# kehanxuuu/vspg-pbrt-v4

Measured on AMD Instinct MI355X. Metric: Mpaths/sec on 1920x1080 homogeneous fog; relMSE vs CPU ref at equal spp, higher is better.
Workload: dtype f32; 1 GPU; fog-box 1920x1080, guidedvolpathvspg vspguiding=true (primary-ray VSP; App. F options), 1 spp per step per GPU, independent sampler seed 0, maxdepth 5

## Files before the change

### vspg-pbrt-v4_amd/csrc/vspg_device.h

```cpp
#pragma once
#include <hip/hip_runtime.h>
#include <stdint.h>

#include "../../include/vspg.h"
#include "vspg_arith.h"
#include "vspg_libm.h"

#define VDEV __device__ __forceinline__
#ifdef VSPG_WF_DEBUG
__device__ unsigned int g_dbg_err[8];
#define VSPG_DBG_CHECK(cond, bit) do { if (!(cond)) atomicOr(&g_dbg_err[0], 1u << (bit)); } while (0)
#else
#define VSPG_DBG_CHECK(cond, bit)
#endif
#ifdef VSPG_NOINLINE_LEAVES
#define VLEAF __device__ __attribute__((noinline))
#else
#define VLEAF __device__ __forceinline__
#endif

VSPG_NS_BEGIN

#ifdef VSPG_PROFILE
enum { PS_INTERSECT = 0, PS_HASHRNG, PS_DIST_GUIDED, PS_DIST_PLAIN, PS_SURF_PRE, PS_NEE, PS_NEE_TR, PS_VOL_SAMPLE,
// ... 360 lines not shown
    V3 local = V3{clampf(sinTheta, -1, 1) * cosPhi, clampf(sinTheta, -1, 1) * sinPhi, clampf(cosTheta, -1, 1)};
    *pdf = henyey_greenstein(cosTheta, g);
    return f.from_local(local);
}
VDEV V3 sample_henyey_greenstein(V3 wo, float g, float u0, float u1, float *pdf) {
    float st, ct;
    float phi = hg_pre(g, u0, u1, &st, &ct);
    float sinPhi, cosPhi;
    sincosf_(phi, &sinPhi, &cosPhi);
    return hg_post(wo, g, st, ct, sinPhi, cosPhi, pdf);
}
VDEV float cos_hemi_pre(float u0, float u1, float *r, bool *degenerate) {
    float ox = 2 * u0 - 1, oy = 2 * u1 - 1;
    *degenerate = (ox == 0 && oy == 0);
    const bool xmajor = __builtin_fabsf(ox) > __builtin_fabsf(oy);
    const float q = (xmajor ? oy : ox) / (xmajor ? ox : oy);
    *r = xmajor ? ox : oy;
    const float t = kPiOver4 * q;
    return xmajor ? t : kPiOver2 - t;
}
VDEV V3 cos_hemi_post(float r, bool degenerate, float sinT, float cosT) {
    float dx = degenerate ? 0.f : r * cosT;
    float dy = degenerate ? 0.f : r * sinT;
    float z = safe_sqrt(1 - sqr(dx) - sqr(dy));
    return V3{dx, dy, z};
}
VDEV V3 sample_cosine_hemisphere(float u0, float u1) {
    float r;
    bool deg;
    float theta = cos_hemi_pre(u0, u1, &r, &deg);
    float sinTheta, cosTheta;
    sincosf_(theta, &sinTheta, &cosTheta);
    return cos_hemi_post(r, deg, sinTheta, cosTheta);
}

struct P3i {
    V3 lo, hi;
    VDEV V3 mid() const { return V3{(lo.x + hi.x) / 2, (lo.y + hi.y) / 2, (lo.z + hi.z) / 2}; }
    VDEV V3 err() const { return V3{(hi.x - lo.x) / 2, (hi.y - lo.y) / 2, (hi.z - lo.z) / 2}; }
};
VDEV P3i p3i_exact(V3 p) { return P3i{p, p}; }
VDEV void interval_ve(float v, float e, float *lo, float *hi) {
    float l = next_float_down(v - e), h = next_float_up(v + e);
    *lo = e == 0 ? v : l;
    *hi = e == 0 ? v : h;
}
VDEV P3i p3i_from_err(V3 p, V3 e) {
    P3i r;
    interval_ve(p.x, e.x, &r.lo.x, &r.hi.x);
    interval_ve(p.y, e.y, &r.lo.y, &r.hi.y);
    interval_ve(p.z, e.z, &r.lo.z, &r.hi.z);
    return r;
}
VDEV float offset_axis(float po, float off) {
    const uint32_t ui = f2b(po), os = f2b(off) & 0x80000000u;
    uint32_t r = ui + ((uint32_t)((int32_t)(ui ^ os) >> 31) | 1u);
    r = (ui << 1) == 0u ? (os | 1u) : r;
    const bool keep = !__builtin_islessgreater(off, 0.f) || (ui ^ os) == 0x7f800000u;
    return b2f(keep ? ui : r);
}
VDEV V3 offset_ray_origin(P3i pi, V3 n, V3 w) {
    float d = dot(vabs(n), pi.err());
    V3 offset = n * d;
    if (dot(w, n) < 0) offset = -offset;
    V3 po = pi.mid() + offset;
    return V3{offset_axis(po.x, offset.x), offset_axis(po.y, offset.y), offset_axis(po.z, offset.z)};
}
VDEV V3 medium_ray_origin(P3i pi) {
    const V3 n = V3{0.f, 0.f, 0.f};
    const float d = dot(n, pi.err());
    return pi.mid() + n * d;
}

#define VSPG_GLOBAL_AS __attribute__((address_space(1)))
struct DQuad {
    float p00[3], p10[3], p01[3], p11[3], e1[3], e2[3];
    float n[3], dpdu_n[3], perr[3];
    float inv_l1, inv_l2, area;
    float Kd[3], Le[3];
    int32_t two_sided, is_light, has_lobes;
    int32_t flags;
};
enum { SURF_INTERFACE = 1, SURF_IFACE_SHIFT = 1 };
enum { kIsectStepsMask = 3, kIsectUvSwapped = 4, kIsectAxisAligned = 8, kIsectAxisShift = 4 };
struct IsectRec {
    float f[14];
    int32_t kind;
    int32_t axes;
};
inline int isect_rec_build(IsectRec *rec, const float *n, const float *p00, const float *e1, const float *e2, float inv_l1, float inv_l2, int cur) {
    int ax[3];
    const float *vec[3] = {n, e1, e2};
    for (int j = 0; j < 3; ++j) {
        int nz = 0;
        ax[j] = -1;
        for (int k = 0; k < 3; ++k)
            if (vec[j][k] != 0) { nz++; ax[j] = k; }
        if (nz != 1) ax[j] = -1;
    }
    const int an = ax[0], a1 = ax[1], a2 = ax[2];
    for (int k = 0; k < 14; ++k) rec->f[k] = 0;
    int frame = 0;
    bool swapped = false;
    if (an >= 0 && an <= 2 && a1 >= 0 && a2 >= 0 && an != a1 && an != a2 && a1 != a2 && (n[an] == 1.0f || n[an] == -1.0f)) {
        swapped = a1 != (an + 1) % 3;
        const int au = swapped ? a2 : a1, av = swapped ? a1 : a2;
        frame = an;
        rec->kind = 1;
        rec->f[0] = n[an]; rec->f[1] = p00[an]; rec->f[2] = p00[au]; rec->f[3] = p00[av];
        rec->f[4] = swapped ? e2[a2] : e1[a1]; rec->f[5] = swapped ? e1[a1] : e2[a2];
        rec->f[6] = swapped ? inv_l2 : inv_l1; rec->f[7] = swapped ? inv_l1 : inv_l2;
    } else {
        rec->kind = 0;
        for (int k = 0; k < 3; ++k) { rec->f[k] = n[k]; rec->f[3 + k] = p00[k]; rec->f[6 + k] = e1[k]; rec->f[9 + k] = e2[k]; }
        rec->f[12] = inv_l1; rec->f[13] = inv_l2;
    }
    if (cur < 0 || cur > 2) cur = 0;
    rec->axes = ((frame - cur + 3) % 3) | (swapped ? kIsectUvSwapped : 0) | (rec->kind == 1 ? kIsectAxisAligned : 0) | (frame << kIsectAxisShift);
    return frame;
}
constexpr int kPlaneChunk = 4;
struct RectPlanes {
    float c[3][kPlaneChunk];
    uint32_t listed, always;
    uint32_t order[4];
};
static_assert(VSPG_MAX_QUADS <= 16 && 3 * kPlaneChunk + VSPG_MAX_QUADS < 32, "a record index is 4 bits of RectPlanes::order, a position one bit of 32");
inline void rect_planes_build(RectPlanes *T, const IsectRec *recs, int n) {
    *T = RectPlanes{};
    uint32_t done = 0;
    int count[3] = {0, 0, 0};
    auto place = [&](int pos, int i) { T->order[(pos - 1) >> 3] |= (uint32_t)i << (4 * ((pos - 1) & 7)); };
    for (int i = 0; i < n; ++i) {
        const int a = (recs[i].axes >> kIsectAxisShift) & 3;
        if (!(recs[i].axes & kIsectAxisAligned) || a > 2 || count[a] == kPlaneChunk) continue;
        const int pos = kPlaneChunk * a + count[a] + 1;
        T->c[a][count[a]++] = recs[i].f[1];
        T->listed |= 1u << pos;
        place(pos, i);
        done |= 1u << i;
    }
    int pos = 3 * kPlaneChunk + 1;
    for (int i = 0; i < n; ++i)
        if (!(done >> i & 1u)) {
            T->always |= 1u << pos;
            place(pos++, i);
        }
}
struct DField {
    int32_t n_nodes, n_regions;
    const VspgKdNode *nodes;
    const VspgFieldRegion *regions;
    const float *aux;
    const float4 *lobes;
};
constexpr int kMaxLights = VSPG_MAX_QUADS + VSPG_MAX_INFINITE_LIGHTS + VSPG_MAX_POINT_LIGHTS;
struct DLightNode {
    float bmin[3], bmax[3], w[3];
    float phi, cosTheta_o, cosTheta_e;
    int32_t twoSided;
    uint32_t child_or_light;
    int32_t is_leaf;
};
struct DLightSampler {
    int32_t mode;
    int32_t n_nodes, n_inf, n_alias;
    DLightNode nodes[2 * kMaxLights];
    int32_t inf_light[VSPG_MAX_INFINITE_LIGHTS];
    uint32_t bit_trail[kMaxLights];
    float alias_p[kMaxLights], alias_q[kMaxLights];
    int32_t alias_i[kMaxLights];
    int32_t light_of_quad[VSPG_MAX_QUADS];
};
struct DTri {
    float p0[3], nx;
    float p1[3], ny;
    float p2[3], nz;
    float dpdu_n[3];
    int32_t id;
    float Kd[3];
    int32_t flags;
};
struct DSphere {
    float m[12], mi[12];
    float radius, thetaZMin, thetaZMax, phiMax;
    float Kd[3];
    int32_t flip, has_lobes, flags;
};
struct DBvh4Node {
    float lox[4], loy[4], loz[4], hix[4], hiy[4], hiz[4];
    int32_t child[4];
    int32_t pad[4];
};
static_assert(sizeof(DBvh4Node) == 128, "one node = eight 16-byte loads");
constexpr int32_t kBvhAbsent = (int32_t)0x80000000;
constexpr int kBvhStack = 48;
struct PixelWindow {
    int32_t x0, y0, x1, y1;
};
__host__ __device__ __forceinline__ int win_tile_x0(const PixelWindow &w) { return w.x0 >> 3; }
__host__ __device__ __forceinline__ int win_tile_y0(const PixelWindow &w) { return w.y0 >> 3; }
__host__ __device__ __forceinline__ int win_tiles_x(const PixelWindow &w) { return ((w.x1 + 7) >> 3) - (w.x0 >> 3); }
__host__ __device__ __forceinline__ int win_tiles_y(const PixelWindow &w) { return ((w.y1 + 7) >> 3) - (w.y0 >> 3); }
__host__ __device__ __forceinline__ bool win_has(const PixelWindow &w, int px, int py) { return px >= w.x0 && px < w.x1 && py >= w.y0 && py < w.y1; }
struct DEnvLight {
    int32_t res;
    float integral;
    float m[9], mi[9];
    float sum_L[3];
    const float *texels;
    const float *func;
    const float *cdf;
    const float *mfunc;
    const float *mcdf;
};
struct DPointLight {
    int32_t type;
    float pos[3];
    float I[3];
    float mi[12];
    float cosFalloffEnd, cosFalloffStart;
    float axis[3];
};
struct DScene {
    int32_t n_quads, n_lights;
    int32_t n_tris, n_bvh_nodes;
    int32_t n_spheres, has_boundaries, camera_in_medium, pad_b;
    VspgCamera cam;
    int32_t medium_type;
    float sigma_a[3], sigma_s[3], Le[3], g;
// ... 84 lines not shown
static_assert(VSPG_MAX_QUADS <= kSpherePrim, "rectangle indices lie below the first sphere primitive");
VDEV bool is_sphere(int prim) { return prim >= kSpherePrim; }
VDEV int sphere_of(int prim) { return prim - kSpherePrim; }

VDEV bool beyond(float num, float denom, float tMax) {
    return __builtin_fabsf(num) > tMax * __builtin_fabsf(denom) * 1.000001f;
}
VDEV float comp(V3 v, int axis) { return axis == 0 ? v.x : (axis == 1 ? v.y : v.z); }
VDEV void swap_regs(float &a, float &b) { asm("v_swap_b32 %0, %1" : "+v"(a), "+v"(b)); }
VDEV void here(float a, float b, float c, float d) { asm volatile("" : : "s"(a), "s"(b), "s"(c), "s"(d)); }
VDEV void rect_frame(V3 &o, V3 &d, int steps) {
#pragma nounroll
    for (int k = steps & kIsectStepsMask; k > 0; --k) {
        swap_regs(o.x, o.y);
        swap_regs(o.y, o.z);
        swap_regs(d.x, d.y);
        swap_regs(d.y, d.z);
    }
}
VDEV bool rect_hit_uv(const IsectRec &r, V3 o, V3 d, float tMax, float *tHit, float *uHit, float *vHit) {
    float num, denom, u, v, t;
    bool cand;
    if (r.axes & kIsectAxisAligned) {
        denom = d.x;
        num = r.f[1] - o.x;
        cand = (int32_t)(__builtin_bit_cast(uint32_t, num) ^ __builtin_bit_cast(uint32_t, denom)) >= 0;
        cand = cand & !beyond(num, denom, tMax);
#if defined(__HIP_DEVICE_COMPILE__)
        const bool some = __ballot(cand) != 0ull;
#elif defined(VSPG_RECT_VOTE_TAKEN)
        const bool some = true;
#else
        const bool some = cand;
#endif
        if (!some) return false;
        t = num / denom;
        cand = cand & (t > 0) & (t < tMax);
        float pu = o.y + d.y * t, pv = o.z + d.z * t;
        u = ((pu - r.f[2]) * r.f[4]) * r.f[6];
        v = ((pv - r.f[3]) * r.f[5]) * r.f[7];
    } else {
        V3 n = V3{r.f[0], r.f[1], r.f[2]}, p00 = V3{r.f[3], r.f[4], r.f[5]};
        denom = dot(n, d);
        num = dot(n, p00 - o);
        cand = ((num > 0) & (denom > 0)) | ((num < 0) & (denom < 0));
        cand = cand & !beyond(num, denom, tMax);
#if defined(__HIP_DEVICE_COMPILE__)
        const bool some = __ballot(cand) != 0ull;
#elif defined(VSPG_RECT_VOTE_TAKEN)
        const bool some = true;
#else
        const bool some = cand;
#endif
        if (!some) return false;
        t = num / denom;
        cand = cand & (t > 0) & (t < tMax);
        V3 p = o + d * t;
        V3 rel = p - p00;
        u = dot(rel, V3{r.f[6], r.f[7], r.f[8]}) * r.f[12];
        v = dot(rel, V3{r.f[9], r.f[10], r.f[11]}) * r.f[13];
    }
    cand = cand & !((u < 0) | (u > 1) | (v < 0) | (v > 1));
    *tHit = t;
    *uHit = u;
    *vHit = v;
    return cand;
}
VDEV bool rects_closest(const IsectRec *recs, int n, V3 o, V3 d, float tMax, float *tBest, int *iBest, float *uBest, float *vBest) {
    bool hit = false;
    float bt = tMax, bu = 0, bv = 0;
    int bi = 0;
    V3 fo = o, fd = d;
    for (int i = 0; i < n; ++i) {
        const IsectRec &r = recs[i];
        float t, u, v;
        rect_frame(fo, fd, r.axes);
        const bool h = rect_hit_uv(r, fo, fd, bt, &t, &u, &v);
        const bool swapped = (r.axes & kIsectUvSwapped) != 0;
        hit = hit | h;
        bt = h ? t : bt;
        bi = h ? i : bi;
        bu = h ? (swapped ? v : u) : bu;
        bv = h ? (swapped ? u : v) : bv;
    }
    *tBest = bt;
    *iBest = bi;
    *uBest = bu;
    *vBest = bv;
    return hit;
}
VDEV bool rects_any(const IsectRec *recs, int n, V3 o, V3 d, float tMax) {
    bool any = false;
    V3 fo = o, fd = d;
    for (int i = 0; i < n; ++i) {
        const IsectRec &r = recs[i];
        float t, u, v;
        rect_frame(fo, fd, r.axes);
        any = any | rect_hit_uv(r, fo, fd, tMax, &t, &u, &v);
    }
    return any;
}
VDEV uint32_t plane_vote(float c, float oa, float da, float thr, uint32_t bit) {
    const float num = c - oa;
    const bool same = (int32_t)(__builtin_bit_cast(uint32_t, num) ^ __builtin_bit_cast(uint32_t, da)) >= 0, within = !(__builtin_fabsf(num) > thr);
#if defined(__HIP_DEVICE_COMPILE__)
    const bool some = (__builtin_amdgcn_ballot_w64(same) & __builtin_amdgcn_ballot_w64(within)) != 0ull;
#elif defined(VSPG_RECT_VOTE_TAKEN)
    const bool some = true;
#else
    const bool some = same & within;
#endif
    return some ? bit : 0u;
}
VDEV uint32_t axis_votes(const float *c, uint32_t listed, int a, float oa, float da, float tMax) {
    const float thr = tMax * __builtin_fabsf(da) * 1.000001f;
    static_assert(kPlaneChunk == 4, "one four-word load");
    const float p[kPlaneChunk] = {c[0], c[1], c[2], c[3]};
    here(p[0], p[1], p[2], p[3]);
    uint32_t m = 0;
#pragma unroll
    for (int k = 0; k < kPlaneChunk; ++k) {
        const uint32_t bit = 2u << (kPlaneChunk * a + k);
        if (!(listed & bit)) return m;
        m |= plane_vote(p[k], oa, da, thr, bit);
    }
    return m;
}
VDEV bool rects_any_planes(const RectPlanes &T, const IsectRec *recs, V3 o, V3 d, float tMax) {
    const uint32_t listed = T.listed;
    uint32_t mask = T.always;
    mask |= axis_votes(T.c[0], listed, 0, o.x, d.x, tMax);
    mask |= axis_votes(T.c[1], listed, 1, o.y, d.y, tMax);
    mask |= axis_votes(T.c[2], listed, 2, o.z, d.z, tMax);
    if (mask == 0) return false;
    bool any = false;
    V3 fo = o, fd = d;
    int cur = 0;
#pragma nounroll
    while (mask != 0) {
        const int pos = __builtin_ctz(mask) - 1;
        mask &= mask - 1;
        const IsectRec &r = recs[(T.order[pos >> 3] >> (4 * (pos & 7))) & 15u];
        const int frame = (r.axes >> kIsectAxisShift) & 3;
        float t, u, v;
        rect_frame(fo, fd, frame - cur + (frame < cur ? 3 : 0));
        cur = frame;
        any = any | rect_hit_uv(r, fo, fd, tMax, &t, &u, &v);
    }
    return any;
}
VDEV bool quad_hit_uv(const DQuad &q, V3 o, V3 d, float tMax, float *tHit, float *uHit, float *vHit) {
    V3 n = ld3(q.n), p00 = ld3(q.p00);
    float denom = dot(n, d);
    float num = dot(n, p00 - o);
    bool cand = (num > 0 && denom > 0) || (num < 0 && denom < 0);
    if (!cand) return false;
    float t = num / denom;
    if (!(t > 0) || !(t < tMax)) return false;
    V3 p = o + d * t;
    V3 rel = p - p00;
    float u = dot(rel, ld3(q.e1)) * q.inv_l1;
    float v = dot(rel, ld3(q.e2)) * q.inv_l2;
    if (u < 0 || u > 1 || v < 0 || v > 1) return false;
    *tHit = t;
    *uHit = u;
    *vHit = v;
// ... 196 lines not shown
        const float *row = S.mi + 4 * k;
        const float v = (row[0] * ro.x + row[1] * ro.y) + (row[2] * ro.z + row[3]);
        const float e = g3 * (__builtin_fabsf(row[0] * ro.x) + __builtin_fabsf(row[1] * ro.y) + __builtin_fabsf(row[2] * ro.z) + __builtin_fabsf(row[3]));
        oi[k] = ivl_from_err(v, e);
        const float ev = g3 * (__builtin_fabsf(row[0] * rd.x) + __builtin_fabsf(row[1] * rd.y) + __builtin_fabsf(row[2] * rd.z));
        const float vv = row[0] * rd.x + row[1] * rd.y + row[2] * rd.z;
        di[k] = ivl_from_err(vv, ev);
    }
    const Ivl a = ivl_add(ivl_add(ivl_sqr(di[0]), ivl_sqr(di[1])), ivl_sqr(di[2]));
    const Ivl b = ivl_fmul(2.f, ivl_add(ivl_add(ivl_mul(di[0], oi[0]), ivl_mul(di[1], oi[1])), ivl_mul(di[2], oi[2])));
    const Ivl c = ivl_sub(ivl_add(ivl_add(ivl_sqr(oi[0]), ivl_sqr(oi[1])), ivl_sqr(oi[2])), ivl_sqr(ivl_x(S.radius)));
    const Ivl f = ivl_div(b, ivl_fmul(2.f, a));
    const Ivl v0 = ivl_sub(oi[0], ivl_mul(f, di[0])), v1 = ivl_sub(oi[1], ivl_mul(f, di[1])), v2 = ivl_sub(oi[2], ivl_mul(f, di[2]));
    const Ivl length = ivl_sqrt(ivl_add(ivl_add(ivl_sqr(v0), ivl_sqr(v1)), ivl_sqr(v2)));
    const Ivl discrim = ivl_mul(ivl_mul(ivl_fmul(4.f, a), ivl_add(ivl_x(S.radius), length)), ivl_sub(ivl_x(S.radius), length));
    if (discrim.lo < 0) return false;
    const Ivl rootDiscrim = ivl_sqrt(discrim);
    Ivl q;
    if (ivl_mid(b) < 0) q = ivl_fmul(-.5f, ivl_sub(b, rootDiscrim));
    else q = ivl_fmul(-.5f, ivl_add(b, rootDiscrim));
    Ivl t0 = ivl_div(q, a), t1 = ivl_div(c, q);
    if (t0.lo > t1.lo) { const Ivl t = t0; t0 = t1; t1 = t; }
    if (t0.hi > tMax || t1.lo <= 0) return false;
    Ivl tShapeHit = t0;
    if (tShapeHit.lo <= 0) {
        tShapeHit = t1;
        if (tShapeHit.hi > tMax) return false;
    }
    const float ts = ivl_mid(tShapeHit);
    V3 pHit = V3{ivl_mid(oi[0]) + ts * ivl_mid(di[0]), ivl_mid(oi[1]) + ts * ivl_mid(di[1]), ivl_mid(oi[2]) + ts * ivl_mid(di[2])};
    const float sc = S.radius / len(pHit);
    pHit = V3{pHit.x * sc, pHit.y * sc, pHit.z * sc};
    if (pHit.x == 0 && pHit.y == 0) pHit.x = 1e-5f * S.radius;
    *tHit = ts;
    *pObj = pHit;
    return true;
}
struct SphereSurf {
    P3i pi;
    V3 n, dpdu_n;
};
template <bool WITH_DPDU = true>
VDEV SphereSurf sphere_interaction(const DSphere &S, V3 pHit) {
    SphereSurf r;
    const float cosTheta = pHit.z / S.radius;
    const float zRadius = __builtin_sqrtf(sqr(pHit.x) + sqr(pHit.y));
    const float cosPhi = pHit.x / zRadius, sinPhi = pHit.y / zRadius;
    const V3 dpdu = V3{-S.phiMax * pHit.y, S.phiMax * pHit.x, 0.f};
    const float sinTheta = safe_sqrt(1 - sqr(cosTheta));
    const float dth = S.thetaZMax - S.thetaZMin;
    const V3 dpdv = V3{dth * (pHit.z * cosPhi), dth * (pHit.z * sinPhi), dth * (-S.radius * sinTheta)};
    V3 no = normalize(cross(dpdu, dpdv));
    if (S.flip) no = -no;
    constexpr float g5 = (5 * kMachineEps) / (1 - 5 * kMachineEps), g3 = (3 * kMachineEps) / (1 - 3 * kMachineEps);
    const Ivl px = ivl_from_err(pHit.x, g5 * __builtin_fabsf(pHit.x)), py = ivl_from_err(pHit.y, g5 * __builtin_fabsf(pHit.y)),
              pz = ivl_from_err(pHit.z, g5 * __builtin_fabsf(pHit.z));
    const float x = ivl_mid(px), y = ivl_mid(py), z = ivl_mid(pz);
    const float ex = (px.hi - px.lo) / 2, ey = (py.hi - py.lo) / 2, ez = (pz.hi - pz.lo) / 2;
    const bool exact = (px.hi - px.lo) == 0 && (py.hi - py.lo) == 0 && (pz.hi - pz.lo) == 0;
    float pv[3], pe[3];
#pragma unroll
    for (int k = 0; k < 3; ++k) {
        const float *row = S.m + 4 * k;
        pv[k] = (row[0] * x + row[1] * y) + (row[2] * z + row[3]);
        const float ea = g3 * (__builtin_fabsf(row[0] * x) + __builtin_fabsf(row[1] * y) + __builtin_fabsf(row[2] * z) + __builtin_fabsf(row[3]));
        pe[k] = exact ? ea : (g3 + 1) * (__builtin_fabsf(row[0]) * ex + __builtin_fabsf(row[1]) * ey + __builtin_fabsf(row[2]) * ez) + ea;
    }
    r.pi = p3i_from_err(V3{pv[0], pv[1], pv[2]}, V3{pe[0], pe[1], pe[2]});
    const float *mi = S.mi;
    r.n = normalize(V3{mi[0] * no.x + mi[4] * no.y + mi[8] * no.z, mi[1] * no.x + mi[5] * no.y + mi[9] * no.z, mi[2] * no.x + mi[6] * no.y + mi[10] * no.z});
    if (WITH_DPDU) {
        const float *m = S.m;
        r.dpdu_n = normalize(V3{m[0] * dpdu.x + m[1] * dpdu.y + m[2] * dpdu.z, m[4] * dpdu.x + m[5] * dpdu.y + m[6] * dpdu.z, m[8] * dpdu.x + m[9] * dpdu.y + m[10] * dpdu.z});
    } else {
        r.dpdu_n = mk(0, 0, 0);
    }
    return r;
}

template <bool FULL = true>
VLEAF Isect scene_intersect(const DScene &S, V3 o, V3 d, float tMax) {
    Isect best;
    float bu, bv;
    best.hit = rects_closest(S.irec, S.n_quads, o, d, tMax, &best.t, &best.quad, &bu, &bv);
    const DQuad &q = quad_at(best.quad);
    best.p = quad_point(q, bu, bv);
    best.n = ld3(q.n);
    if (FULL && S.n_tris > 0) {
        int tp = 0;
        TriHit h;
        if (bvh_closest(S, o, d, best.t, &tp, &h)) {
            const DTri &T = S.tris[tp];
            best.hit = true;
            best.t = h.t;
            best.quad = -2 - tp;
            best.p = V3{h.b0, h.b1, h.b2};
            best.n = V3{T.nx, T.ny, T.nz};
        }
    }
    if (FULL && S.n_spheres > 0) {
        for (int i = 0; i < S.n_spheres; ++i) {
            float t;
            V3 pObj;
            if (sphere_intersect(S.spheres[i], o, d, tMax, &t, &pObj) && t < best.t) {
                best.hit = true;
                best.t = t;
                best.quad = kSpherePrim + i;
                best.p = pObj;
                best.n = sphere_interaction<false>(S.spheres[i], pObj).n;
            }
        }
    }
    return best;
}
template <bool FULL = true>
VLEAF bool scene_intersect_any(const DScene &S, V3 o, V3 d, float tMax) {
    bool any = rects_any_planes(S.planes, S.irec, o, d, tMax);
    if (FULL && S.n_tris > 0 && !any) any = bvh_any(S, o, d, tMax);
    if (FULL && S.n_spheres > 0 && !any) {
        for (int i = 0; i < S.n_spheres; ++i) {
            float t;
            V3 pObj;
            any = any || sphere_intersect(S.spheres[i], o, d, tMax, &t, &pObj);
        }
    }
    return any;
}
VDEV int surf_flags(const DScene &S, int prim) {
    if (is_tri(prim)) return S.tris[tri_of(prim)].flags;
    if (is_sphere(prim)) return S.spheres[sphere_of(prim)].flags;
    return quad_at(prim).flags;
}
VDEV P3i tri_pi(const DTri &T, V3 b) {
    const V3 p0 = ld3(T.p0), p1 = ld3(T.p1), p2 = ld3(T.p2);
    const V3 p = p0 * b.x + p1 * b.y + p2 * b.z;
    const V3 s = vabs(p0 * b.x) + vabs(p1 * b.y) + vabs(p2 * b.z);
    constexpr float g7 = (7 * kMachineEps) / (1 - 7 * kMachineEps);
    return p3i_from_err(p, V3{g7 * s.x, g7 * s.y, g7 * s.z});
}
template <bool FULL = true>
VDEV P3i surf_pi(const DScene &S, int prim, V3 p) {
    if (FULL && is_sphere(prim)) return sphere_interaction<false>(S.spheres[sphere_of(prim)], p).pi;
    if (FULL && is_tri(prim)) return tri_pi(S.tris[tri_of(prim)], p);
    return p3i_from_err(p, ld3(quad_at(prim).perr));
}
VDEV float dot_vn(V3 v, V3 n) {
    const float cd = n.z * v.z;
    const float sop = __builtin_fmaf(n.y, v.y, cd);
    const float err = __builtin_fmaf(n.z, v.z, -cd);
    return __builtin_fmaf(n.x, v.x, sop + err);
}
VDEV bool get_medium(int flags, V3 n, V3 w, bool medium) {
    const int iface = flags >> SURF_IFACE_SHIFT;
    if (iface) return dot_vn(w, n) > 0 ? (iface & VSPG_IFACE_OUTSIDE) != 0 : (iface & VSPG_IFACE_INSIDE) != 0;
    return medium;
}

struct MediumProps {
    Spec sigma_a, sigma_s, Le;
    float g;
    Spec sigma_t;
    float bb_temp = 0.f, bb_scale = 0.f;
};
struct MajSeg {
    float tMin, tMax;
    Spec sigma_maj;
};
// ... 619 lines not shown
```

### vspg-pbrt-v4_amd/csrc/vspg_scene_build.hip

```cpp
#include "vspg_scene_build.h"

#include <algorithm>
#include <cmath>
#include <cstdlib>
#include <cstring>
#include <string>

#include "vspg_error.h"

namespace vspg_host {

PcgJump pcg_jump(unsigned long long delta) {
    unsigned long long curMult = 0x5851f42d4c957f2dULL, curPlus = 1u, accMult = 1u, accPlus = 0u;
    while (delta > 0) {
        if (delta & 1) {
            accMult *= curMult;
            accPlus = accPlus * curMult + curPlus;
        }
        curPlus = (curMult + 1) * curPlus;
        curMult *= curMult;
        delta /= 2;
    }
    return PcgJump{accMult, accPlus};
}
// ... 347 lines not shown
        d[i] = sum / 3;
        for (int c = 0; c < 3; ++c) sumL[c] += rgb[3 * i + c] > 0.f ? rgb[3 * i + c] : 0.f;
    }
    for (int c = 0; c < 3; ++c) T->sum_L[c] = sumL[c];
    double acc = 0.;
    for (size_t i = 0; i < n; ++i) acc += d[i];
    const float average = (float)(acc / (double)n);
    bool all_zero = true;
    for (size_t i = 0; i < n; ++i) {
        const float v = d[i] - average;
        d[i] = v < 0.f ? 0.f : v;
        all_zero = all_zero && d[i] == 0;
    }
    if (all_zero) for (size_t i = 0; i < n; ++i) d[i] = 1.f;
    float *cdf = T->buf.data() + T->o_cdf, *mfunc = T->buf.data() + T->o_mfunc, *mcdf = T->buf.data() + T->o_mcdf;
    for (int v = 0; v < res; ++v) mfunc[v] = env_build_1d(d + (size_t)v * res, cdf + (size_t)v * (res + 1), res);
    T->integral = env_build_1d(mfunc, mcdf, res);
}
bool env_matrices(const float *m34, float *m, float *mi) {
    static const float ident[12] = {1, 0, 0, 0, 0, 1, 0, 0, 0, 0, 1, 0};
    const float *s = m34 ? m34 : ident;
    double A[9];
    for (int r = 0; r < 3; ++r)
        for (int c = 0; c < 3; ++c) {
            m[3 * r + c] = s[4 * r + c];
            A[3 * r + c] = (double)s[4 * r + c];
            if (!std::isfinite(s[4 * r + c])) return false;
        }
    const double a = A[0], b = A[1], c = A[2], d = A[3], e = A[4], f = A[5], g = A[6], h = A[7], i = A[8];
    const double c00 = e * i - f * h, c01 = f * g - d * i, c02 = d * h - e * g;
    const double det = (a * c00 + b * c01) + c * c02;
    if (!(det != 0) || !std::isfinite(det)) return false;
    const double adj[9] = {c00, c * h - b * i, b * f - c * e, c01, a * i - c * g, c * d - a * f, c02, b * g - a * h, a * e - b * d};
    for (int k = 0; k < 9; ++k) {
        mi[k] = (float)(adj[k] / det);
        if (!std::isfinite(mi[k])) return false;
    }
    return true;
}
static int32_t surf_flags_of(int material, int medium_interface) {
    const int b = medium_interface & (VSPG_IFACE_INSIDE | VSPG_IFACE_OUTSIDE);
    const int iface = (b == VSPG_IFACE_INSIDE || b == VSPG_IFACE_OUTSIDE) ? b : 0;
    return (material == VSPG_MATERIAL_INTERFACE ? SURF_INTERFACE : 0) | (iface << SURF_IFACE_SHIFT);
}
void build_dscene(const VspgScene &sc, const VspgIntegratorParams &prm, const VspgRenderConfig &cfg, DScene *D) {
    using namespace hostmath;
    memset(D, 0, sizeof *D);
    D->n_quads = sc.n_quads;
    int frame = 0;
    for (int i = 0; i < sc.n_quads; ++i) {
        const VspgQuad &in = sc.quads[i];
        DQuad &q = D->quads[i];
        H3 p00 = ld(in.p00), e1 = ld(in.e1), e2 = ld(in.e2);
        H3 p10 = add(p00, e1), p01 = add(p00, e2), p11 = add(p10, e2);
        stv(q.p00, p00); stv(q.p10, p10); stv(q.p01, p01); stv(q.p11, p11); stv(q.e1, e1); stv(q.e2, e2);
        H3 c = crossv(e1, e2);
        q.area = std::sqrt(len2v(c));
        H3 n = normv(c);
        if (in.reverse_orientation) n = H3{-n.x, -n.y, -n.z};
        stv(q.n, n);
        stv(q.dpdu_n, normv(e1));
        const float eps = 0x1p-24f;
        float g6 = (6 * eps) / (1 - 6 * eps);
        H3 s = add(add(absv(p00), absv(p01)), add(absv(p10), absv(p11)));
        stv(q.perr, H3{s.x * g6, s.y * g6, s.z * g6});
        q.inv_l1 = 1.f / len2v(e1);
        q.inv_l2 = 1.f / len2v(e2);
        bool lobes = false, light = false;
        for (int k = 0; k < 3; ++k) {
            float kd = in.Kd[k];
            kd = kd < 0 ? 0 : (kd > 1 ? 1 : kd);
            q.Kd[k] = kd;
            q.Le[k] = in.Le[k];
            lobes = lobes || kd != 0;
            light = light || in.Le[k] != 0;
        }
        q.two_sided = in.two_sided;
        q.is_light = light;
        q.has_lobes = lobes;
        q.flags = surf_flags_of(in.material, in.medium_interface);
        frame = isect_rec_build(&D->irec[i], q.n, q.p00, q.e1, q.e2, q.inv_l1, q.inv_l2, frame);
        if (light) D->light_quads[D->n_lights++] = i;
    }
    rect_planes_build(&D->planes, D->irec, D->n_quads);
    D->n_inf = sc.n_infinite_lights;
    for (int i = 0; i < sc.n_infinite_lights && i < VSPG_MAX_INFINITE_LIGHTS; ++i) {
        D->inf_type[i] = sc.infinite_lights[i].type;
        for (int k = 0; k < 3; ++k) { D->inf_L[i][k] = sc.infinite_lights[i].L[k]; D->inf_w[i][k] = sc.infinite_lights[i].w_light[k]; }
        if (D->inf_type[i] == VSPG_LIGHT_IMAGE_INFINITE) {
            DEnvLight &E = D->env[i];
            E.res = 1;
            for (int k = 0; k < 3; ++k) { E.m[4 * k] = E.mi[4 * k] = 1.f; E.sum_L[k] = 1.f; }
        }
    }
    D->n_point = sc.n_point_lights;
    for (int i = 0; i < sc.n_point_lights && i < VSPG_MAX_POINT_LIGHTS; ++i) {
        const VspgPointLight &in = sc.point_lights[i];
        DPointLight &P = D->point[i];
        P.type = in.type;
        const float *m = in.render_from_light;
        float q[4];
        for (int k = 0; k < 4; ++k) {
            volatile float a = m[4 * k] * 0.f;
            volatile float b = m[4 * k + 1] * 0.f;
            volatile float c2 = m[4 * k + 2] * 0.f;
            volatile float sum = a + b;
            sum = sum + c2;
            sum = sum + m[4 * k + 3];
            q[k] = sum;
        }
        for (int k = 0; k < 3; ++k) P.pos[k] = q[3] == 1 ? q[k] : q[k] / q[3];
        for (int k = 0; k < 3; ++k) P.I[k] = in.I[k];
        for (int k = 0; k < 12; ++k) P.mi[k] = in.light_from_render[k];
        P.cosFalloffEnd = P.cosFalloffStart = 0.f;
        P.axis[0] = P.axis[1] = 0.f; P.axis[2] = 1.f;
        if (in.type == VSPG_LIGHT_SPOT) {
            volatile float start_deg = in.cone_angle_deg - in.cone_delta_deg;
            const float deg2rad = 3.14159265358979323846f / 180;
            volatile float rad_end = deg2rad * in.cone_angle_deg, rad_start = deg2rad * start_deg;
            P.cosFalloffEnd = std::cos((float)rad_end);
            P.cosFalloffStart = std::cos((float)rad_start);
            float w[3];
            for (int k = 0; k < 3; ++k) {
                volatile float a = m[4 * k] * 0.f;
                volatile float b = m[4 * k + 1] * 0.f;
                volatile float c2 = m[4 * k + 2] * 1.f;
                volatile float sum = a + b;
                sum = sum + c2;
                w[k] = sum;
            }
            stv(P.axis, normv(H3{w[0], w[1], w[2]}));
        }
    }
    {
        float lo[3] = {kInf, kInf, kInf}, hi[3] = {-kInf, -kInf, -kInf};
        auto grow = [&](const float *q) { for (int k = 0; k < 3; ++k) { lo[k] = q[k] < lo[k] ? q[k] : lo[k]; hi[k] = q[k] > hi[k] ? q[k] : hi[k]; } };
        for (int i = 0; i < D->n_quads; ++i) { grow(D->quads[i].p00); grow(D->quads[i].p10); grow(D->quads[i].p01); grow(D->quads[i].p11); }
        for (int i = 0; i < sc.n_triangles && sc.tri_p; ++i) {
            DTri T;
            if (derive_triangle(sc.tri_p + 9 * (size_t)i, nullptr, i, &T)) { grow(T.p0); grow(T.p1); grow(T.p2); }
        }
        for (int i = 0; i < sc.n_spheres; ++i) {
            const float *m = sc.spheres[i].render_from_object, rr = sc.spheres[i].radius;
            for (int c = 0; c < 8; ++c) {
                const float x = (c & 1) ? rr : -rr, y = (c & 2) ? rr : -rr, z = (c & 4) ? rr : -rr;
                float q[3];
                for (int k = 0; k < 3; ++k) {
                    volatile float a = m[4 * k] * x;
                    volatile float b = m[4 * k + 1] * y;
                    volatile float c2 = m[4 * k + 2] * z;
                    volatile float sum = a + b;
                    sum = sum + c2;
                    sum = sum + m[4 * k + 3];
                    q[k] = sum;
                }
                grow(q);
            }
        }
        D->scene_radius = 0.f;
        if (lo[0] <= hi[0]) {
            volatile float cx = (lo[0] + hi[0]) / 2, cy = (lo[1] + hi[1]) / 2, cz = (lo[2] + hi[2]) / 2;
            volatile float dx = cx - hi[0], dy = cy - hi[1], dz = cz - hi[2];
            volatile float l2 = dx * dx;
            l2 = l2 + dy * dy;
            l2 = l2 + dz * dz;
            D->scene_radius = std::sqrt(l2);
// ... 438 lines not shown
```

Before: 4145 Mpaths/s.

## Merge paired axis-aligned parallel rect tests into one twin intersection

At scene build time, adjacent axis-aligned quads that share the same axis and the same in-plane bounds (such as the opposite faces of a box) are marked as twins, and the second plane offset is stored in the first record. The closest-hit loop then tests both planes with one divide and one bounds check when the whole wavefront sees at most one candidate, and skips the second record. It also returns early when no lane in the wavefront has a candidate. This is meant to cut per-ray ALU work for fog-box style scenes, at the cost of extra wavefront ballots and divergent branches inside the intersection loop.

```diff
diff --git a/vspg-pbrt-v4_amd/csrc/vspg_device.h b/vspg-pbrt-v4_amd/csrc/vspg_device.h
--- a/vspg-pbrt-v4_amd/csrc/vspg_device.h
+++ b/vspg-pbrt-v4_amd/csrc/vspg_device.h
@@ -466,7 +466,7 @@
     int32_t flags;
 };
 enum { SURF_INTERFACE = 1, SURF_IFACE_SHIFT = 1 };
-enum { kIsectStepsMask = 3, kIsectUvSwapped = 4, kIsectAxisAligned = 8, kIsectAxisShift = 4 };
+enum { kIsectStepsMask = 3, kIsectUvSwapped = 4, kIsectAxisAligned = 8, kIsectAxisShift = 4, kIsectTwin = 64, kIsectTwinSwapped = 128 };
 struct IsectRec {
     float f[14];
     int32_t kind;
@@ -530,6 +530,18 @@
             T->always |= 1u << pos;
             place(pos++, i);
         }
+}
+inline void rect_twins_mark(IsectRec *recs, int n) {
+    for (int i = 0; i + 1 < n; ++i) {
+        IsectRec &a = recs[i];
+        const IsectRec &b = recs[i + 1];
+        if (a.axes & kIsectTwin) { ++i; continue; }
+        if (!(a.axes & kIsectAxisAligned) || !(b.axes & kIsectAxisAligned) || (b.axes & (kIsectStepsMask | kIsectTwin))) continue;
+        if ((((a.axes ^ b.axes) >> kIsectAxisShift) & 3) || __builtin_memcmp(&a.f[2], &b.f[2], 6 * sizeof(float)) != 0) continue;
+        a.axes |= kIsectTwin | ((b.axes & kIsectUvSwapped) ? kIsectTwinSwapped : 0);
+        a.f[8] = b.f[1];
+        ++i;
+    }
 }
 struct DField {
     int32_t n_nodes, n_regions;
@@ -780,6 +792,82 @@
         bi = h ? i : bi;
         bu = h ? (swapped ? v : u) : bu;
         bv = h ? (swapped ? u : v) : bv;
+    }
+    *tBest = bt;
+    *iBest = bi;
+    *uBest = bu;
+    *vBest = bv;
+    return hit;
+}
+#if defined(__HIP_DEVICE_COMPILE__) || !defined(VSPG_RECT_TWIN_PATH)
+#undef VSPG_RECT_TWIN_PATH
+#define VSPG_RECT_TWIN_PATH(fallback)
+#endif
+VDEV bool rect_hit_uv_twins(const IsectRec &r, V3 o, V3 d, float tMax, float *tHit, float *uHit, float *vHit, bool *second, bool *merged) {
+    const float denom = d.x;
+    float num = r.f[1] - o.x;
+    bool cand = (int32_t)(__builtin_bit_cast(uint32_t, num) ^ __builtin_bit_cast(uint32_t, denom)) >= 0;
+    cand = cand & !beyond(num, denom, tMax);
+    bool sel = false, two = false;
+    if (r.axes & kIsectTwin) {
+        const float numB = r.f[8] - o.x;
+        bool candB = (int32_t)(__builtin_bit_cast(uint32_t, numB) ^ __builtin_bit_cast(uint32_t, denom)) >= 0;
+        candB = candB & !beyond(numB, denom, tMax);
+#if defined(__HIP_DEVICE_COMPILE__)
+        const bool both = __builtin_amdgcn_ballot_w64(cand & candB) != 0ull;
+#elif VSPG_RECT_TWIN_VOTE == 2
+        const bool both = true;
+#else
+        const bool both = cand & candB;
+#endif
+        VSPG_RECT_TWIN_PATH(both);
+        if (!both) {
+            two = true;
+            sel = candB;
+            num = sel ? numB : num;
+            cand = cand | candB;
+        }
+    }
+    *second = sel;
+    *merged = two;
+#if defined(__HIP_DEVICE_COMPILE__)
+    const bool some = __builtin_amdgcn_ballot_w64(cand) != 0ull;
+#elif VSPG_RECT_TWIN_VOTE == 1
+    const bool some = true;
+#else
+    const bool some = cand;
+#endif
+    if (!some) return false;
+    const float t = num / denom;
+    cand = cand & (t > 0) & (t < tMax);
+    const float pu = o.y + d.y * t, pv = o.z + d.z * t;
+    const float u = ((pu - r.f[2]) * r.f[4]) * r.f[6];
+    const float v = ((pv - r.f[3]) * r.f[5]) * r.f[7];
+    cand = cand & !((u < 0) | (u > 1) | (v < 0) | (v > 1));
+    *tHit = t;
+    *uHit = u;
+    *vHit = v;
+    return cand;
+}
+VDEV bool rects_closest_twins(const IsectRec *recs, int n, V3 o, V3 d, float tMax, float *tBest, int *iBest, float *uBest, float *vBest) {
+    bool hit = false;
+    float bt = tMax, bu = 0, bv = 0;
+    int bi = 0;
+    V3 fo = o, fd = d;
+    for (int i = 0; i < n;) {
+        const IsectRec &r = recs[i];
+        float t, u, v;
+        bool second = false, merged = false, h;
+        rect_frame(fo, fd, r.axes);
+        if (r.axes & kIsectAxisAligned) h = rect_hit_uv_twins(r, fo, fd, bt, &t, &u, &v, &second, &merged);
+        else h = rect_hit_uv(r, fo, fd, bt, &t, &u, &v);
+        const bool swapped = second ? (r.axes & kIsectTwinSwapped) != 0 : (r.axes & kIsectUvSwapped) != 0;
+        hit = hit | h;
+        bt = h ? t : bt;
+        bi = h ? i + (second ? 1 : 0) : bi;
+        bu = h ? (swapped ? v : u) : bu;
+        bv = h ? (swapped ? u : v) : bv;
+        i += merged ? 2 : 1;
     }
     *tBest = bt;
     *iBest = bi;
@@ -1142,7 +1230,7 @@
 VLEAF Isect scene_intersect(const DScene &S, V3 o, V3 d, float tMax) {
     Isect best;
     float bu, bv;
-    best.hit = rects_closest(S.irec, S.n_quads, o, d, tMax, &best.t, &best.quad, &bu, &bv);
+    best.hit = rects_closest_twins(S.irec, S.n_quads, o, d, tMax, &best.t, &best.quad, &bu, &bv);
     const DQuad &q = quad_at(best.quad);
     best.p = quad_point(q, bu, bv);
     best.n = ld3(q.n);
diff --git a/vspg-pbrt-v4_amd/csrc/vspg_scene_build.hip b/vspg-pbrt-v4_amd/csrc/vspg_scene_build.hip
--- a/vspg-pbrt-v4_amd/csrc/vspg_scene_build.hip
+++ b/vspg-pbrt-v4_amd/csrc/vspg_scene_build.hip
@@ -453,6 +453,7 @@
         frame = isect_rec_build(&D->irec[i], q.n, q.p00, q.e1, q.e2, q.inv_l1, q.inv_l2, frame);
         if (light) D->light_quads[D->n_lights++] = i;
     }
+    rect_twins_mark(D->irec, D->n_quads);
     rect_planes_build(&D->planes, D->irec, D->n_quads);
     D->n_inf = sc.n_infinite_lights;
     for (int i = 0; i < sc.n_infinite_lights && i < VSPG_MAX_INFINITE_LIGHTS; ++i) {
```

After: 4197 Mpaths/s (median of 6 runs). 1.01x the previous value.
